# tsinghua-fib-lab/CLSR

Hardware: AMD Instinct MI355X
Metric: train interactions/sec @ batch 4096 seq_len 50 (higher is better)
Workload: dtype f32 (every product at fp32 accuracy: fp32-input MFMAs or three bf16 pieces per operand; the two-piece split-product step is precision_modes.fp32x3)

## Files before the change

### clsr_amd/csrc/linear.hip

```cpp
#include <stdlib.h>
#include "common.h"
#include "clsr_hip.h"
#include <cstdlib>

struct PGemmArgs {
  const float* X; int ldx;
  int T; int G;
  const float* Xmul; int ldmul;
  const float* in_scale; const float* in_shift; int in_relu;
  const float* Wt; int Kp;
  int ldw;
  const float* bias;
  const float* addU; int ldu;
  const float* addV; int ldv;
  float* Y; int ldy; int accumulate;
  double* stats;
  int M, K, N;
  const float* ez; int ldez; const float* e_scale; const float* e_shift; const float* e_mean; const float* e_invstd;
  int no_ring;
  int no_compact;
  int rm_tc, rm_T, rm_t0;
};

__device__ __forceinline__ int range_row(int v, int rm_tc, int rm_T, int rm_t0) {
  if (rm_tc == 0) return v;
  const int q = (int)((unsigned)v / (unsigned)rm_tc);
  return q * rm_T + rm_t0 + (v - q * rm_tc);
}

template <int OT, bool STATS>
__global__ void __launch_bounds__(256) pgemm_generic_kernel(PGemmArgs a) {
  extern __shared__ __attribute__((aligned(16))) float lds[];
  const int tid = threadIdx.x, wave = tid >> 6, lane = tid & 63;
  const int j = lane & 15, g = lane >> 4;
  const int ntile_out = (a.N + 15) >> 4;
// ... 701 lines not shown
  for (int e = blockIdx.x * 256 + threadIdx.x; e < total; e += gridDim.x * 256) {
    const int o = e / d.I, i = e - o * d.I;
    float v = d.s1 * (d.transposed ? d.src1[(long)o * d.ld1 + i] : d.src1[(long)i * d.ld1 + o]);
    if (d.src2) v += d.s2 * (d.transposed ? d.src2[(long)o * d.ld2 + i] : d.src2[(long)i * d.ld2 + o]);
    d.dst[(long)(d.o0 + o) * d.Kp + d.i0 + i] = v;
  }
}

extern "C" int clsr_sizeof_pack_desc(void) { return (int)sizeof(clsr_pack_desc); }

extern "C" int clsr_pack_batch(const clsr_pack_desc* descs_device, int n, int max_elems, void* stream) {
  CLSR_CHECK_ARG(descs_device && n > 0 && max_elems > 0);
  int bx = clsr_cdiv(max_elems, 256);
  if (bx > 64) bx = 64;
  hipLaunchKernelGGL(pack_batch_kernel, dim3(bx, n), dim3(256), 0, (hipStream_t)stream, descs_device);
  CLSR_CHECK_LAUNCH();
  return CLSR_OK;
}

#define DW_T CLSR_DW_T
#define DW_CHUNK CLSR_DW_CHUNK

struct DwArgs {
  const void* X; int ldx; int T; int G; const float* Xmul; int ldmul;
  const float* in_scale; const float* in_shift; int in_relu;
  const void* dY; int ldy;
  float* partial;
  int M, K, N;
  int rm_tc, rm_T, rm_t0, pstride, poff;
};

#define DW_W (16 * DW_T)
#define DW_LDS_FLOATS (64 * 2 * DW_W > 2 * DW_CHUNK ? 64 * 2 * DW_W : 2 * DW_CHUNK)
template <int MODE, bool XH = false, bool YH = false, int KTC = 0, int NTC = 0>
__device__ __forceinline__ void dw_body(const DwArgs& a, float* lds, const int bx, const int gx, const int by,
                                        const int bz, const int gz) {
  float* Xs = lds;
  float* Ys = lds + 64 * DW_W;
  const int tid = threadIdx.x, wave = tid >> 6, lane = tid & 63;
  const int i = lane & 15, g = lane >> 4;
  const int k0 = by * DW_W, n0 = bz * DW_W;
  const int ktc = KTC ? KTC : min(DW_T, ((a.K + 15) >> 4) - by * DW_T);
  const int ntc = NTC ? NTC : min(DW_T, ((a.N + 15) >> 4) - bz * DW_T);
  const int kmax4 = ((a.K + 3) & ~3) - 4, nmax4 = a.N - 4;

  f32x4 acc[DW_T][DW_T];
#pragma unroll
  for (int kt = 0; kt < DW_T; ++kt)
#pragma unroll
    for (int nt = 0; nt < DW_T; ++nt) acc[kt][nt] = (f32x4){0.f, 0.f, 0.f, 0.f};
  float bsum[DW_T];
#pragma unroll
  for (int nt = 0; nt < DW_T; ++nt) bsum[nt] = 0.f;

  constexpr int Q = DW_W / 4;
  constexpr int NLD = 64 * Q / 256;
  f32x4 xr[NLD], yr[NLD], mr[MODE == 1 ? NLD : 1];
  unsigned vmask = 0;
  f32x4 scv[MODE == 2 ? NLD : 1], shv[MODE == 2 ? NLD : 1];
  if (MODE == 2) {
#pragma unroll
    for (int j = 0; j < NLD; ++j) {
      const int idx = tid + 256 * j;
      const int c4 = idx - (idx / Q) * Q;
      int kcol = k0 + 4 * c4;
      kcol = kcol <= kmax4 ? kcol : kmax4;
      scv[j] = ld4(a.in_scale + kcol);
// ... 12 lines not shown
      m = range_row(m < a.M ? m : a.M - 1, a.rm_tc, a.rm_T, a.rm_t0);
      int kcol = k0 + 4 * c4, ncol = n0 + 4 * c4;
      if (mv && kcol <= kmax4) vmask |= 1u << j;
      if (mv && ncol <= nmax4) vmask |= 1u << (8 + j);
      kcol = kcol <= kmax4 ? kcol : kmax4;
      ncol = ncol <= nmax4 ? ncol : nmax4;
      long xrow = m, r = m;
      if (a.T > 0) {
        const unsigned rr = (unsigned)m / (unsigned)a.T;
        r = rr;
        if (a.G > 0) xrow = (long)(rr / (unsigned)a.G) * a.T + (m - (int)rr * a.T);
      }
      xr[j] = load4e<XH>(a.X, xrow * a.ldx + kcol);
      if (MODE == 1) mr[j] = ld4(a.Xmul + r * a.ldmul + kcol);
      yr[j] = load4e<YH>(a.dY, (long)m * a.ldy + ncol);
    }
  };
  auto stage = [&]() {
    const f32x4 z = {0.f, 0.f, 0.f, 0.f};
#pragma unroll
    for (int j = 0; j < NLD; ++j) {
      const int idx = tid + 256 * j;
      f32x4 xv = xr[j];
      if (MODE == 1) xv *= mr[j];
      if (MODE == 2) {
        xv = xv * scv[j] + shv[j];
        if (a.in_relu) { xv.x = fmaxf(xv.x, 0.f); xv.y = fmaxf(xv.y, 0.f); xv.z = fmaxf(xv.z, 0.f); xv.w = fmaxf(xv.w, 0.f); }
      }
      st4(Xs + 4 * idx, (vmask >> j) & 1u ? xv : z);
      st4(Ys + 4 * idx, (vmask >> (8 + j)) & 1u ? yr[j] : z);
    }
  };

  fetch(bx);
  for (int tile = bx; tile < ntiles; tile += gx) {
    __syncthreads();
    stage();
    __syncthreads();
    fetch(tile + gx);
    const float* xw = Xs + (16 * wave + g) * DW_W + i;
    const float* yw = Ys + (16 * wave + g) * DW_W + i;
#pragma unroll
    for (int s = 0; s < 4; ++s) {
      float av[DW_T], bv[DW_T];
#pragma unroll
      for (int t = 0; t < DW_T; ++t) {
        av[t] = xw[(4 * s) * DW_W + 16 * t];
        bv[t] = yw[(4 * s) * DW_W + 16 * t];
      }
#pragma unroll
      for (int kt = 0; kt < DW_T; ++kt)
        if (kt < ktc) {
#pragma unroll
          for (int nt = 0; nt < DW_T; ++nt)
            if (nt < ntc) MFMA4(acc[kt][nt], av[kt], bv[nt]);
        }
#pragma unroll
      for (int nt = 0; nt < DW_T; ++nt) bsum[nt] += bv[nt];
    }
  }
#pragma unroll
  for (int nt = 0; nt < DW_T; ++nt) bsum[nt] = col4_sum(bsum[nt]);
  __syncthreads();
  float* red = lds;

  auto store_to = [&](float* dst) {
// ... 8 lines not shown
    if (g == 0) {
#pragma unroll
      for (int nt = 0; nt < DW_T; ++nt) dst[DW_T * DW_T * 256 + nt * 16 + i] = bsum[nt];
    }
  };
  auto add_from = [&](const float* src) {
#pragma unroll
    for (int kt = 0; kt < DW_T; ++kt)
#pragma unroll
      for (int nt = 0; nt < DW_T; ++nt) {
        const float* t = src + (kt * DW_T + nt) * 256 + (4 * g) * 16 + i;
        acc[kt][nt] += (f32x4){t[0], t[16], t[32], t[48]};
      }
#pragma unroll
    for (int nt = 0; nt < DW_T; ++nt) bsum[nt] += src[DW_T * DW_T * 256 + nt * 16 + i];
  };
  if (wave >= 2) store_to(red + (wave - 2) * DW_CHUNK);
  __syncthreads();
  if (wave < 2) add_from(red + wave * DW_CHUNK);
  __syncthreads();
  if (wave == 1) store_to(red);
  __syncthreads();
  if (wave == 0) {
    add_from(red);
    const long chunk = (long)by * gz + bz;
    store_to(a.partial + (chunk * a.pstride + a.poff + bx) * DW_CHUNK);
  }
}

template <int MODE, bool XH = false, bool YH = false, int KTC = 0, int NTC = 0>
__global__ void __launch_bounds__(256) pgemm_dw_kernel(DwArgs a) {
  __shared__ __attribute__((aligned(16))) float lds[DW_LDS_FLOATS];
  dw_body<MODE, XH, YH, KTC, NTC>(a, lds, blockIdx.x, gridDim.x, blockIdx.y, blockIdx.z, gridDim.z);
}

#define DWM_MAX 12
struct DwMultiArgs {
  DwArgs d[DWM_MAX];
  int first[DWM_MAX + 1];
  int gx[DWM_MAX];
  short nch[DWM_MAX];
  short mode[DWM_MAX];
  int n;
  int spec;
};
__global__ void __launch_bounds__(256) dw_multi_kernel(DwMultiArgs m) {
  __shared__ __attribute__((aligned(16))) float lds[DW_LDS_FLOATS];
  int j = 0;
  while (j + 1 < m.n && (int)blockIdx.x >= m.first[j + 1]) ++j;
  const int local = blockIdx.x - m.first[j];
  const int gx = m.gx[j], nch = m.nch[j];
  const int bx = local % gx, c = local / gx;
  const int by = c / nch, bz = c - by * nch;
  const int ktc = min(DW_T, ((m.d[j].K + 15) >> 4) - by * DW_T), ntc = min(DW_T, ((m.d[j].N + 15) >> 4) - bz * DW_T);
  if (m.mode[j] == 0) {
    if (m.spec && ktc == 3 && ntc == 5) dw_body<0, false, false, 3, 5>(m.d[j], lds, bx, gx, by, bz, nch);
    else if (m.spec && ktc == 5 && ntc == 5) dw_body<0, false, false, 5, 5>(m.d[j], lds, bx, gx, by, bz, nch);
    else if (m.spec > 1 && ktc == 5 && ntc == 3) dw_body<0, false, false, 5, 3>(m.d[j], lds, bx, gx, by, bz, nch);
    else dw_body<0>(m.d[j], lds, bx, gx, by, bz, nch);
  } else if (m.mode[j] == 1) {
    if (m.spec > 1 && ktc == 3 && ntc == 3) dw_body<1, false, false, 3, 3>(m.d[j], lds, bx, gx, by, bz, nch);
    else dw_body<1>(m.d[j], lds, bx, gx, by, bz, nch);
  } else dw_body<2>(m.d[j], lds, bx, gx, by, bz, nch);
}

__global__ void __launch_bounds__(1024) dw_reduce_kernel(const float* __restrict__ partial, int nparts, int K,
                                                        int N, int kchunks, int nchunks, float scale,
                                                        float* __restrict__ dW, int ldw,
                                                        float* __restrict__ db, int accumulate) {
  __shared__ float red[16][64];
  const int total = K * N + (db ? N : 0);
  const int e = blockIdx.x * 64 + (threadIdx.x & 63);
  const int sub = threadIdx.x >> 6;
  float s = 0.f;
  float* o = nullptr;
  if (e < total) {
    const float* p;
    if (e < K * N) {
      const int k = e / N, n = e - k * N;
      const int kc = k / (16 * DW_T), nc = n / (16 * DW_T);
      const int kk = k - kc * 16 * DW_T, nn = n - nc * 16 * DW_T;
      const long off = ((kk >> 4) * DW_T + (nn >> 4)) * 256 + (kk & 15) * 16 + (nn & 15);
      p = partial + ((long)(kc * nchunks + nc) * nparts) * DW_CHUNK + off;
      o = dW + (long)k * ldw + n;
    } else {
      const int n = e - K * N;
      const int nc = n / (16 * DW_T), nn = n - nc * 16 * DW_T;
      p = partial + ((long)nc * nparts) * DW_CHUNK + DW_T * DW_T * 256 + nn;
      o = db + n;
    }
    for (int w = sub; w < nparts; w += 16) s += p[(long)w * DW_CHUNK];
  }
  red[sub][threadIdx.x & 63] = s;
  __syncthreads();
  if (sub == 0 && e < total) {
    s = 0.f;
#pragma unroll
    for (int u = 0; u < 16; ++u) s += red[u][threadIdx.x];
    s *= scale;
    *o = accumulate ? *o + s : s;
  }
}

static int dw_grid_x(int M) {
  int tiles = clsr_cdiv(M, 64);
  int gx = clsr_cdiv(tiles, 4);
  constexpr int cap = 512;
  if (gx > cap) gx = cap;
  if (gx < 1) gx = 1;
  return gx;
}

extern "C" long clsr_pgemm_dw_workspace_floats(int M, int K, int N) {
  const long chunks = (long)clsr_cdiv(K, 16 * DW_T) * clsr_cdiv(N, 16 * DW_T);
  return chunks * dw_grid_x(M) * DW_CHUNK;
}

static int dw_launch_partial(const void* X, int ldx, int T, int G, const float* Xmul, int ldmul,
                             const float* in_scale, const float* in_shift, int in_relu, const void* dY, int ldy,
                             int M, int K, int N, float* workspace, hipStream_t s, int* gx_out, int x_bf16 = 0,
                             int dy_bf16 = 0) {
  CLSR_CHECK_ARG(X && dY && workspace && M >= 0 && K > 0 && N > 0);
  CLSR_CHECK_ARG(!(in_scale && !in_shift));
  CLSR_CHECK_SUPPORTED(N % 4 == 0 && ldx % 4 == 0 && ldy % 4 == 0 && ldx >= ((K + 3) & ~3) &&
                       (!Xmul || (ldmul % 4 == 0 && ldmul >= ((K + 3) & ~3))) &&
                       ((uintptr_t)X % 16) == 0 && ((uintptr_t)dY % 16) == 0);
  DwArgs a;
  a.X = X; a.ldx = ldx; a.T = T; a.G = G; a.Xmul = Xmul; a.ldmul = ldmul;
  a.in_scale = in_scale; a.in_shift = in_shift; a.in_relu = in_relu;
  a.dY = dY; a.ldy = ldy; a.partial = workspace; a.M = M; a.K = K; a.N = N;
  const int kch = clsr_cdiv(K, 16 * DW_T), nch = clsr_cdiv(N, 16 * DW_T);
  const int gx = dw_grid_x(M);
  a.rm_tc = a.rm_T = a.rm_t0 = 0; a.pstride = gx; a.poff = 0;
  CLSR_CHECK_SUPPORTED(!(Xmul && in_scale) && !(in_scale && K % 4));
  if (x_bf16 || dy_bf16) {
    CLSR_CHECK_SUPPORTED(dy_bf16 && ((x_bf16 && in_scale) || (!x_bf16 && Xmul)));
    if (x_bf16) hipLaunchKernelGGL((pgemm_dw_kernel<2, true, true>), dim3(gx, kch, nch), dim3(256), 0, s, a);
    else hipLaunchKernelGGL((pgemm_dw_kernel<1, false, true>), dim3(gx, kch, nch), dim3(256), 0, s, a);
    CLSR_CHECK_LAUNCH();
    *gx_out = gx;
    return CLSR_OK;
  }
  const int ktn = clsr_cdiv(K, 16), ntn = clsr_cdiv(N, 16);
  const bool one = kch == 1 && nch == 1;
#define DW_SPEC(MD, KT_, NT_)                                                                                          \
  if (one && ktn == KT_ && ntn == NT_) {                                                                               \
    hipLaunchKernelGGL((pgemm_dw_kernel<MD, false, false, KT_, NT_>), dim3(gx, 1, 1), dim3(256), 0, s, a);            \
    CLSR_CHECK_LAUNCH();                                                                                               \
    *gx_out = gx;                                                                                                      \
    return CLSR_OK;                                                                                                    \
  }
  if (Xmul) { DW_SPEC(1, 5, 5) DW_SPEC(1, 3, 3) }
  else if (in_scale) { DW_SPEC(2, 5, 3) DW_SPEC(2, 5, 5) }
  else { DW_SPEC(0, 5, 5) DW_SPEC(0, 3, 5) DW_SPEC(0, 3, 3) DW_SPEC(0, 5, 3) }
#undef DW_SPEC
  if (Xmul) hipLaunchKernelGGL(pgemm_dw_kernel<1>, dim3(gx, kch, nch), dim3(256), 0, s, a);
  else if (in_scale) hipLaunchKernelGGL(pgemm_dw_kernel<2>, dim3(gx, kch, nch), dim3(256), 0, s, a);
  else hipLaunchKernelGGL(pgemm_dw_kernel<0>, dim3(gx, kch, nch), dim3(256), 0, s, a);
  CLSR_CHECK_LAUNCH();
  *gx_out = gx;
  return CLSR_OK;
}

extern "C" int clsr_sizeof_dwjob(void) { return (int)sizeof(clsr_dwjob); }

extern "C" int clsr_pgemm_dw_partial_multi(const clsr_dwjob* jobs, int n, void* stream) {
  CLSR_CHECK_ARG(jobs && n > 0 && n <= DWM_MAX);
  DwMultiArgs m;
  m.n = n;
  int total = 0;
  for (int j = 0; j < n; ++j) {
    const clsr_dwjob& q = jobs[j];
    CLSR_CHECK_ARG(q.X && q.dY && q.workspace && q.M > 0 && q.K > 0 && q.N > 0 && !(q.in_scale && !q.in_shift));
    CLSR_CHECK_SUPPORTED(!q.x_bf16 && !q.dy_bf16);
    CLSR_CHECK_SUPPORTED(q.N % 4 == 0 && q.ldx % 4 == 0 && q.ldy % 4 == 0 && q.ldx >= ((q.K + 3) & ~3) &&
                         (!q.Xmul || (q.ldmul % 4 == 0 && q.ldmul >= ((q.K + 3) & ~3))) &&
                         ((uintptr_t)q.X % 16) == 0 && ((uintptr_t)q.dY % 16) == 0);
    CLSR_CHECK_SUPPORTED(!(q.Xmul && q.in_scale) && !(q.in_scale && q.K % 4));
    DwArgs& a = m.d[j];
    a.X = q.X; a.ldx = q.ldx; a.T = q.T; a.G = q.G; a.Xmul = q.Xmul; a.ldmul = q.ldmul;
    a.in_scale = q.in_scale; a.in_shift = q.in_shift; a.in_relu = q.in_relu;
    a.dY = q.dY; a.ldy = q.ldy; a.partial = q.workspace; a.M = q.M; a.K = q.K; a.N = q.N;
    const int kch = clsr_cdiv(q.K, 16 * DW_T), nch = clsr_cdiv(q.N, 16 * DW_T);
    m.first[j] = total;
    m.gx[j] = q.pgx > 0 ? q.pgx : dw_grid_x(q.M);
    CLSR_CHECK_ARG(q.rm_tc >= 0 && (q.rm_tc == 0 || (q.rm_T >= q.rm_t0 + q.rm_tc && q.rm_t0 >= 0 && q.M % q.rm_tc == 0 && !q.T)));
    CLSR_CHECK_ARG(q.pstride == 0 || (q.poff >= 0 && q.poff + m.gx[j] <= q.pstride));
    a.rm_tc = q.rm_tc; a.rm_T = q.rm_T; a.rm_t0 = q.rm_t0;
    a.pstride = q.pstride > 0 ? q.pstride : m.gx[j]; a.poff = q.pstride > 0 ? q.poff : 0;
    m.nch[j] = (short)nch;
    m.mode[j] = (short)(q.Xmul ? 1 : (q.in_scale ? 2 : 0));
    total += m.gx[j] * kch * nch;
  }
  m.first[n] = total;
  m.spec = 2;
  hipLaunchKernelGGL(dw_multi_kernel, dim3(total), dim3(256), 0, (hipStream_t)stream, m);
  CLSR_CHECK_LAUNCH();
  return CLSR_OK;
}

extern "C" int clsr_pgemm_dw(const float* X, int ldx, int T, int G, const float* Xmul, int ldmul,
                             const float* in_scale, const float* in_shift, int in_relu,
                             const float* dY, int ldy, int M, int K, int N, float scale, float* dW,
                             int ldw, float* db, int accumulate, float* workspace, void* stream) {
  CLSR_CHECK_ARG(dW && ldw >= N);
  hipStream_t s = (hipStream_t)stream;
  int gx = 0;
  int rc = dw_launch_partial(X, ldx, T, G, Xmul, ldmul, in_scale, in_shift, in_relu, dY, ldy, M, K, N, workspace, s,
                             &gx);
  if (rc) return rc;
  const int kch = clsr_cdiv(K, 16 * DW_T), nch = clsr_cdiv(N, 16 * DW_T);
  const int total = K * N + (db ? N : 0);
  hipLaunchKernelGGL(dw_reduce_kernel, dim3(clsr_cdiv(total, 64)), dim3(1024), 0, s, workspace, gx, K, N, kch,
                     nch, scale, dW, ldw, db, accumulate);
  CLSR_CHECK_LAUNCH();
  return CLSR_OK;
}

extern "C" int clsr_pgemm_dw_partial(const float* X, int ldx, int T, int G, const float* Xmul, int ldmul,
                                     const float* in_scale, const float* in_shift, int in_relu,
                                     const float* dY, int ldy, int M, int K, int N, float* workspace,
                                     void* stream) {
  int gx = 0;
  return dw_launch_partial(X, ldx, T, G, Xmul, ldmul, in_scale, in_shift, in_relu, dY, ldy, M, K, N, workspace,
                           (hipStream_t)stream, &gx);
}

extern "C" int clsr_pgemm_dw_partial_h(const void* X, int x_bf16, int ldx, int T, int G, const float* Xmul, int ldmul,
                                       const float* in_scale, const float* in_shift, int in_relu,
                                       const void* dY, int dy_bf16, int ldy, int M, int K, int N, float* workspace,
                                       void* stream) {
  int gx = 0;
  return dw_launch_partial(X, ldx, T, G, Xmul, ldmul, in_scale, in_shift, in_relu, dY, ldy, M, K, N, workspace,
                           (hipStream_t)stream, &gx, x_bf16, dy_bf16);
}

extern "C" int clsr_pgemm_dw_parts(int M) { return dw_grid_x(M); }
extern "C" int clsr_sizeof_dw_desc(void) { return (int)sizeof(clsr_dw_desc); }

__global__ void __launch_bounds__(1024) dw_reduce_batch_kernel(const clsr_dw_desc* __restrict__ descs) {
  __shared__ float red[16][64];
  const clsr_dw_desc d = descs[blockIdx.y];
  const int K = d.K, N = d.N;
  const int lane = threadIdx.x & 63, sub = threadIdx.x >> 6;
  const int ktiles = (K + 15) >> 4, ntiles = (N + 15) >> 4;
  const int nchunks = (N + 16 * DW_T - 1) / (16 * DW_T);
  const int wq = ktiles * ntiles * 4;
  const int items = wq + (d.db ? (N + 63) / 64 : 0);
  for (int it = blockIdx.x; it < items; it += gridDim.x) {
    float s = 0.f;
    float* o = nullptr;
    const float* p = nullptr;
    const float* p2 = nullptr;
    if (it < wq) {
      const int tile = it >> 2, q = it & 3;
      const int ktg = tile / ntiles, ntg = tile - ktg * ntiles;
      const int kc = ktg / DW_T, kt = ktg - kc * DW_T, nc = ntg / DW_T, nt = ntg - nc * DW_T;
      const int w = q * 64 + lane;
// ... 45 lines not shown
```

### clsr_amd/net.py

```python
import math
import contextlib
import os
import warnings
from collections import OrderedDict

import numpy as np
import torch

from clsr_amd import ops
from clsr_amd.ops import call, query
from clsr_amd.params import CL, TABLES, UNUSED_TABLE, init_tensor, param_specs

BN_MOMENTUM = 0.95
BN_EPS = 1e-4
F32 = torch.float32


def _pad4(n):
    return (n + 3) // 4 * 4


TF_OPTIMIZERS = {
    "sgd": (0, ()), "gd": (0, ()), "pgd": (0, ()),
    "adagrad": (1, (("accumulator", 0.1),)), "padagrad": (2, (("accumulator", 0.1),)),
# ... 79 lines not shown
        self.att_hist_bwd_pieces = 3 if self.exact_products else 2
        self.bf16_chain = self.precision == "bf16" and os.environ.get("CLSR_BF16_CHAIN", "x1") == "x1"
        self._cur_descs_h = []
        self._plans, self._plan_keep, self._cur_descs = {}, [], []
        self._sort_bytes = {}
        self._ws_tag = ""
        self._side = _SIDE_STREAMS.setdefault(str(torch.device(device)), {})
        self._dense_fork = None
        self._dw_async = False
        self.split_query = True
        self.split_query_min = 16
        self.use_plans = not os.environ.get("CLSR_NO_PLAN")
        self._step_plans = {}
        self._dw_batch = None
        self._buf_allocs = 0
        self.stream_alias = {"@aux": "@lt"}
        self.side_priority = 0
        self.dw_priority = 0
        self.rnn_products = os.environ.get("CLSR_RNN_PRODUCTS", "x6" if self.exact_products else "x3")
        if self.rnn_products not in ("x6", "fp32") + (() if self.exact_products else ("x3",)):
            raise ValueError("CLSR_RNN_PRODUCTS must be 'x6' or 'fp32' (precision='fp32'), also 'x3' otherwise")
        if self.rnn_products == "x6" and max(self.H, self.Du) > 48:
            self.rnn_products = "fp32"
        self.rnn_fused_proj = self.rnn_products in ("x3", "x6") and not os.environ.get("CLSR_NO_RNN_FUSED_PROJ")
        self.proj_gate_pieces = 3 if self.exact_products else 2
        self.proj_bwd_pieces = 3 if self.exact_products else 2
        self.proj_wide_pieces = (2 if self.precision == "bf16" else 3)
        self.rnn_act_tiled = self.rnn_products in ("x3", "x6")
        self.set_att_bwd(os.environ.get("CLSR_ATT_BWD", "x6l1" if self.exact_products else "x3"))
        self.heads_fused = not os.environ.get("CLSR_NO_HEADS_FUSED")
        self.dw_wide = True
        self.dw_wide_entry = (("clsr_pgemm_dw_wide" if os.environ.get("CLSR_DW_WIDE", "x6") == "fp32" else "clsr_pgemm_dw_wide_x6")
                              if self.exact_products else "clsr_pgemm_dw_wide_x3")
        self._dw_batch_wide = None
        self._heads_defer = False
        self._early_lists = None
        self.heads_comm = None
        self._defer_logit_out = False
        self.fold_hist_shares = not os.environ.get("CLSR_NO_FOLD_SHARES")
        self._fold_args, self._folded = None, False
        self.early_user_update = not os.environ.get("CLSR_NO_EARLY_USER_UPDATE")
        self._updated_early = set()
        self._joins = []
        self._dw_pending, self._dw_tables, self._dw_after, self._rp_pending = {}, {}, {}, {}
        self.defer_dw = True
        self.overlap = not os.environ.get("CLSR_NO_OVERLAP")
        self.det_grads = not os.environ.get("CLSR_NO_DET_GRADS")
        self.adam_state = torch.tensor([0.0, 1.0, 1.0, 0.0, 0.0, 0.0, 0.0, 0.0], dtype=torch.float64, device=self.device)
        self.stats24 = torch.zeros(24, dtype=torch.float64, device=self.device)
        self.sumsq_tab, self.losses = self.stats24[:16], self.stats24[16:]
        self.ucount = torch.zeros(1, dtype=F32, device=self.device)
        self.last_shape = None
        self._counts_zeroed = self._ucount_zeroed = self._ticked = False
        self.dp_world = 1
        self.dp_stats_hook = None
        self.dp_comm = None
        self.dp_hooks = None
        self.capture_grads = False
        self.captured = None
        self._aborted = None

    def set_att_bwd(self, mode):
        if mode not in ("x6", "x6l1", "fp32") + (() if self.exact_products else ("x3",)):
            raise ValueError("CLSR_ATT_BWD must be 'x6', 'x6l1' or 'fp32' (precision='fp32'), also 'x3' otherwise")
        self.att_bwd_l0 = "fp32" if mode == "x6l1" else mode
        self.att_bwd = "x6" if mode == "x6l1" else mode
# ... 21 lines not shown
            bad.append("contrastive_loss must be bpr or triplet")
        D = hp.item_embedding_dim + hp.cate_embedding_dim
        if hp.hidden_size != D or hp.user_embedding_dim != D:
            bad.append("hidden_size and user_embedding_dim must equal item+cate dims (alpha fusion, clsr.py:265)")
        bad += self._shape_limits(hp, rnn=True)
        if self.precision == "bf16":
            att = [int(w) for w in hp.att_fcn_layer_sizes]
            qs = (int(hp.user_embedding_dim), int(hp.user_embedding_dim) + D)
            if any(w % 8 for w in att) or any(q % 8 for q in qs) or int(hp.hidden_size) % 8:
                bad.append("precision='bf16' needs att_fcn_layer_sizes %r, the attention query widths %r and hidden_size "
                           "%d to be multiples of 8 (use precision='fp32')" % (att, qs, int(hp.hidden_size)))
        if bad:
            raise NotImplementedError("CLSR HIP path does not support: " + "; ".join(bad))

    @staticmethod
    def _shape_limits(hp, rnn):
        bad = []
        Di, Dc = int(hp.item_embedding_dim), int(hp.cate_embedding_dim)
        if Di % 4 or Dc % 4 or Di <= 0 or Dc <= 0 or Di + Dc > 256:
            bad.append("item / cate embedding dims must be positive multiples of 4, at most 256 together")
        if rnn and (int(hp.hidden_size) % 4 or not 4 <= int(hp.hidden_size) <= 128):
            bad.append("hidden_size must be a multiple of 4 in 4..128")
        if int(hp.max_seq_length) > 256:
            bad.append("max_seq_length must be at most 256")
        widths = list(hp.layer_sizes) + list(getattr(hp, "att_fcn_layer_sizes", None) or [])
        if any(int(w) % 4 or not 4 <= int(w) <= 1024 for w in widths):
            bad.append("MLP layer widths must be multiples of 4 in 4..1024")
        if any(int(w) > 256 for w in (getattr(hp, "att_fcn_layer_sizes", None) or [])):
            bad.append("att_fcn_layer_sizes must be at most 256 wide")
        return bad

    _SWITCHES = ("precision", "table_bf16", "exact_products", "x3", "bf16", "overlap", "defer_dw", "det_grads", "lazy",
                 "use_plans", "heads_fused", "early_user_update", "fold_hist_shares", "enc_x6", "rnn_products", "rnn_fused_proj",
                 "rnn_act_tiled", "att_bwd", "att_bwd_l0", "_l1x", "_l0x", "bf16_chain", "dw_wide", "dw_wide_entry", "split_query",
                 "split_query_min", "rowlist_min_elems", "att_hist_bwd_pieces", "proj_gate_pieces", "proj_bwd_pieces",
                 "proj_wide_pieces")

    def _plan_key(self, what, f):
        hp = self.hp
        g = lambda k: getattr(hp, k, None)
        return (what, id(f), ops.stream_ptr(), self.dp_world, id(self.dp_hooks), id(self.dp_stats_hook), self.dp_comm, self.heads_comm,
                getattr(self, "dp_generation", 0)) + tuple(getattr(self, n, None) for n in self._SWITCHES) + (
                g("learning_rate"), g("embed_l2"), g("layer_l2"), g("embed_l1"), g("layer_l1"), g("max_grad_norm"), g("is_clip_norm"),
                g("discrepancy_loss_weight"), g("contrastive_loss_weight"), g("triplet_margin"),
                g("contrastive_length_threshold"), g("manual_alpha_value"))

    def _planned(self, what, f, run):
        if (not self.use_plans) or self.capture_grads or ops.recording():
            return run()
        key = self._plan_key(what, f)
        ent = self._step_plans.get(key)
        if ent is None:
            self._step_plans[key] = [f, None]
            return run()
        if ent[1] is None:
            plan = ops.record_begin()
            try:
                plan.result = run()
            finally:
                ops.record_end()
            ent[1] = plan
            ent.append(self.last_shape)
            return plan.result
        ops.replay(ent[1])
        self.last_shape = ent[2]
        return ent[1].result

# ... 366 lines not shown
            self._dw_flush()

    def _dw_wide(self, X, ldx, Xmul, ldmul, dY, ldy, M, K, N, dW, ldw, db, acc):
        key = "dww_ws%s.%d.%d.%x" % (self._ws_tag, K, N, dW.data_ptr())
        ws = self._buf(key, query("clsr_pgemm_dw_wide_workspace_floats", M, K, N))
        job = (X, ldx, Xmul, ldmul, dY, ldy, M, K, N, ws, dW, ldw, db, acc)
        if self._dw_batch is not None:
            self._dw_batch_wide.append(job)
            return
        side = None
        if self.overlap and self._ws_tag == "":
            side = self._side_stream("@dw0")
            ops.stream_wait(side, self._fork_point())
            self._dw_async = True
        call(self.dw_wide_entry, *job, stream=side.cuda_stream if side is not None else None)

    @contextlib.contextmanager
    def _dw_batched(self, late=False):
        if not self.defer_dw or self._dw_batch is not None:
            yield
            return
        fork = self._fork_point()
        allocs = self._buf_allocs
        self._dw_batch, self._dw_batch_wide = [], []
        try:
            yield
        finally:
            jobs, self._dw_batch = self._dw_batch, None
            wide, self._dw_batch_wide = self._dw_batch_wide, None
        if not jobs and not wide:
            return
        if late or self._buf_allocs != allocs:
            fork = self._fork_point()
        name = "clsr_hdw_partial_multi" if self.bf16 else "clsr_pgemm_dw_partial_multi"
        if self.overlap and self._ws_tag == "":
            side = self._side_stream("@dw0")
            ops.stream_wait(side, fork)
            if jobs:
                ops.dw_multi(name, jobs, stream=side.cuda_stream)
            for job in wide:
                call(self.dw_wide_entry, *job, stream=side.cuda_stream)
            self._dw_async = True
        else:
            if jobs:
                ops.dw_multi(name, jobs)
            for job in wide:
                call(self.dw_wide_entry, *job)

    def _dw_parts_query(self, any_bf16=False):
        return "clsr_hdw_parts" if self.bf16 else "clsr_pgemm_dw_parts"

    def _dw_launch(self, X, x_bf16, ldx, T, G, Xmul, ldmul, sc, sh, dY, dy_bf16, ldy, M, K, N, ws, stream):
        if self.bf16:
            call("clsr_hdw_partial", X, x_bf16, ldx, T, G, Xmul, ldmul, sc, sh, 1, dY, dy_bf16, ldy, M, K, N, ws,
                 stream=stream)
        elif x_bf16 or dy_bf16:
            call("clsr_pgemm_dw_partial_h", X, x_bf16, ldx, T, G, Xmul, ldmul, sc, sh, 1, dY, dy_bf16, ldy, M, K, N, ws,
                 stream=stream)
        else:
            call("clsr_pgemm_dw_partial", X, ldx, T, G, Xmul, ldmul, sc, sh, 1, dY, ldy, M, K, N, ws, stream=stream)

    def _dw_fused(self, ws, parts, K, N, dW, ldw, db=None, acc=0):
        self._dw_pending.setdefault(self._ws_tag, []).append(
            (ws.data_ptr(), dW.data_ptr(), db.data_ptr() if db is not None else 0, 1.0, parts, K, N, ldw, acc))
        if not self.defer_dw:
            self._dw_flush()

    def _rp(self, partial, parts, stride, n, out):
        self._rp_pending.setdefault(self._ws_tag, []).append(
            (partial.data_ptr(), out.data_ptr(), 1.0, parts, stride, n, 0, 0))

    def _dw_flush(self, tag=None):
        tag = self._ws_tag if tag is None else tag
        pend = self._dw_pending.pop(tag, [])
        if tag == "" and self._dw_async:
            cur = ops.current_stream()
            side = self._side.get("@dw0")
            if side is not None and side.cuda_stream != cur.cuda_stream:
                ops.stream_wait(cur, ops.event_record(side))
            self._dw_async = False
        if pend:
            sig = tuple(pend)
            tab = self._dw_tables.get(sig)
            if tab is None:
                tab = self._dw_tables[sig] = ops.dw_table(sig, self.device)
            call("clsr_dw_reduce_batch", tab[0], tab[1], tab[2])
        rp = self._rp_pending.pop(tag, [])
        if rp:
            ops.multi("clsr_reduce_parts_multi", ops.RpDesc, rp)
        for fn in self._dw_after.pop(tag, []):
            fn()

    def _stats_buf(self, M, N):
# ... 1590 lines not shown
            ops.multi("clsr_tables_reg_multi" + self._th, ops.TableDesc, sweep, l2e, l1e, self.ucount, self.losses[1:])
        if self.capture_grads:
            self.captured = dict(dense={n: g.detach().clone() for n, g in self.Gd.items()},
                                 tables={k: g.detach().clone() for k, g in tg.items()},
                                 dense_sumsq=self.dense_sumsq.clone(), table_sumsq=ss.clone())
            call("clsr_adam_tick", self.adam_state, float(hp.learning_rate), 0.9, 0.999)
            self._dense_update(clip)
        if not tick_early:
            self._join()
        rest = []
        for key, partner, slot, dscale, dloss_scale, dloss, base, nsum in spec:
            V, C = tb[key].shape
            if key in lists and self.tf_opt is not None:
                ids, count, cap = lists[key]
                call("clsr_table_tf_rows", self.tf_opt[0], tb[key], tg[key], self.tab_m.get(key), self.tab_v.get(key),
                     fl[key], ids, count, cap, C, ss[base:], 2, nsum, clip, self.adam_state, lr)
            elif key in lists and self.lazy:
                ids, count, cap = lists[key]
                call("clsr_table_adam_rows" + self._th, tb[key], tg[key], self.tab_m[key], self.tab_v[key], fl[key], ids, count,
                     cap, C, ss[base:], 2, nsum, clip, self.adam_state, 0.9, 0.999, 1e-8)
            elif key in lists:
                call("clsr_table_adam" + self._th, tb[key], tg[key], self.tab_m[key], self.tab_v[key], fl[key], V, C, ss[base:],
                     2, nsum, clip, self.adam_state, 0.9, 0.999, 1e-8, self.lazy)
            else:
                rest.append(key)
        if rest:
            self._tables_update_multi([r for r in sweep if r[0] in {tb[k].data_ptr() for k in rest}], clip)
        if tick_early:
            self._join()

    def precision_note(self):
        if self.precision == "fp32":
            return ("all tensors fp32; EVERY product at fp32 accuracy: v_mfma_f32_16x16x4_f32 (bit-exact fp32 fma chains: recurrences, "
                    "layer-0 forward, heads, encoder-side weight gradients) or three bf16 pieces per operand on "
                    "v_mfma_f32_16x16x32_bf16 with fp32 accumulation (2^-23 relative: history-level attention forward / backward, "
                    "layer-1 forward, the attention-MLP backward with its folded weight gradients%s, the Time4LSTM time-gate "
                    "projection); no two-piece (2^-16) product anywhere" % ("" if self.att_bwd == "x6" else " [CLSR_ATT_BWD=fp32: fp32 MFMAs]"))
        if self.precision == "fp32x3":
            return ("all tensors fp32 (storage, statistics, losses, optimiser exactly as in the fp32 mode); forward products in front "
                    "of a batch-norm + ReLU at fp32 accuracy; the recurrences' hidden products, the attention-MLP backward with its "
                    "folded weight gradients, the history-level attention backward and the fused encoder tail as TWO-piece split-bf16 "
                    "sums hi*hi + hi*lo + lo*hi on v_mfma_f32_16x16x32_bf16 with fp32 accumulation (2^-16 relative per product "
                    "term: narrower than the reference's fp32 products)")
        return ("attention-block activations at (row, step) level (z0, z1, dz0) stored as bf16, their products with ONE bf16 piece per "
                "operand on v_mfma_f32_16x16x32_bf16 with fp32 accumulation"
                + (" (the parity mode's chain kernels with the weight gradients folded in, csrc/attbwdx3.hip)" if self.bf16_chain
                   else " (position-tiled csrc/hgemm.hip kernels, CLSR_BF16_CHAIN=old)")
                + "; history- and row-level tensors, batch-norm statistics, softmax, recurrences, losses, gradients of the "
                "parameters and the optimiser stay fp32")

    def bench_att_layer0(self, f, time_kernel):
        B, T, G, Hn = self.last_shape
        Qs, A0 = self.Du + self.D, self.A0
        run = self._att_layer0_launcher("st", Hn, G, T, Qs)
        t_mm = time_kernel(run)
        flops = 2.0 * B * T * Qs * A0
        bf = self.precision == "bf16"
        peak = 2500.0 if bf else 157.3
        if bf and self._bf16_chain_ok(G, Qs):
            nbytes = float(B) * T * A0 * 2 + float(Hn) * T * (Qs + A0) * 4 + float(B) * (Qs + A0) * 4
            return dict(bound="hbm", kernel="att_l0_fwd_kernel<5,5,1,bf16> (short-term attention layer 0, one wave per history, one "
                                            "bf16 piece per operand, bf16 z0)",
                        achieved=round(nbytes / t_mm / 1e9, 1), peak=8000.0, unit="GB/s", frac=round(nbytes / t_mm / 8e12, 4),
                        bytes_per_launch=nbytes, us_per_launch=round(t_mm * 1e6, 2),
                        formula="B*T*A0*2 (bf16 z0 written) + Hn*T*(Q + A0)*4 (a, U read) + B*(Q + A0)*4 (q, V read)",
                        mfma_tflops=round(flops / t_mm / 1e12, 2))
        return dict(bound="mfma", kernel=(("hgemm_l0g_kernel (short-term attention layer 0, bf16 MFMA, one wave per history group)"
                                           if query("clsr_hgemm_l0_group_supported", G, Qs, A0) else
                                           "hgemm_kernel<MUL,UV> (short-term attention layer 0, bf16 MFMA)") if bf else
                                          "att_l0_fwd_kernel<5,5> (short-term attention layer 0, one wave per history)"
# ... 114 lines not shown
```

### include/clsr_hip.h

```cpp
#ifndef CLSR_HIP_H
#define CLSR_HIP_H
#include <stddef.h>
#ifdef __cplusplus
extern "C" {
#endif

int clsr_version(void);
int clsr_last_error(char* buf, size_t n);

int clsr_graph_begin(void* stream);
int clsr_graph_end(void* stream, void** graph_exec_out);
int clsr_graph_launch(void* graph_exec, void* stream);
int clsr_graph_destroy(void* graph_exec);

int clsr_gather_hist_fwd(const float* item_tbl, const float* cate_tbl, const int* item_idx,
                         const int* cate_idx, long idx_row_stride, const int* seq_len, int len_stride,
                         int Hn, int T, int Di, int Dc, int recent_k, float* hist, float* hist_mean,
                         float* hist_recent, void* stream);
int clsr_gather_hist_fwd_h(const void* item_tbl, const void* cate_tbl, const int* item_idx,
                           const int* cate_idx, long idx_row_stride, const int* seq_len, int len_stride,
                           int Hn, int T, int Di, int Dc, int recent_k, void* hist, int hist_bf16,
                           float* hist_mean, float* hist_recent, void* stream);
int clsr_gather_rows(const float* tbl, const int* idx, long idx_stride, int N, int C, float* out,
                     int ldo, int col0, void* stream);
// ... 273 lines not shown
int clsr_hgemm_l0_group_stats_parts(long Hn);
int clsr_hgemm_l0_group(const float* a, int lda, const float* q, int ldq, const void* Wt, int Kp,
                        const float* U, int ldu, const float* V, int ldv, void* z0, int ldz, double* stats,
                        long Hn, int G, int T, int Q, int A0, void* stream);
int clsr_hgemm_hf32(const void* X, int ldx, const void* Wt, int Kp, float* Y, int ldy, int accumulate,
                    int M, int K, int N, void* stream);
int clsr_pgemm_stats_parts(int M);
int clsr_pgemm_range(const float* X, int ldx, const float* Wt, int Kp, const float* bias, float* Y, int ldy,
                     int accumulate, int Hn, int T, int t0, int t1, int K, int N, void* stream);
int clsr_pgemm(const float* X, int ldx, int T, int G, const float* Xmul, int ldmul,
               const float* in_scale, const float* in_shift, int in_relu, const float* Wt, int Kp,
               const float* bias, const float* addU, int ldu, const float* addV, int ldv, float* Y,
               int ldy, int accumulate, double* stats, int M, int K, int N, void* stream);
int clsr_pgemm_bnbwd(const float* X, int ldx, const float* Wt, int Kp, float* Y, int ldy, const float* z,
                     int ldz, const float* scale, const float* shift, const float* mean, const float* invstd,
                     double* stats, int M, int K, int N, void* stream);
long clsr_pgemm_dw_workspace_floats(int M, int K, int N);
int clsr_pgemm_dw(const float* X, int ldx, int T, int G, const float* Xmul, int ldmul,
                  const float* in_scale, const float* in_shift, int in_relu, const float* dY, int ldy,
                  int M, int K, int N, float scale, float* dW, int ldw, float* db, int accumulate,
                  float* workspace, void* stream);
typedef struct clsr_dw_desc {
  const float* partial; float* dW; float* db;
  float scale;
  int nparts; int K; int N; int ldw; int accumulate;
  const float* partial2; float scale2; int nparts2;
} clsr_dw_desc;
int clsr_sizeof_dw_desc(void);
int clsr_pgemm_dw_parts(int M);
int clsr_hdw_parts(int M);
int clsr_pgemm_dw_partial(const float* X, int ldx, int T, int G, const float* Xmul, int ldmul,
                          const float* in_scale, const float* in_shift, int in_relu, const float* dY, int ldy,
                          int M, int K, int N, float* workspace, void* stream);
int clsr_dw_reduce_batch(const clsr_dw_desc* descs_device, int n, int max_outputs, void* stream);

int clsr_sum_parts_d(const double* partial, int nparts, int n, double* out, void* stream);
int clsr_bn_finalize(const double* stats_partial, int nparts, int C, double count, const float* gamma,
                     const float* beta, float* moving_mean, float* moving_var, float momentum, float eps,
                     int training, float* scale, float* shift, float* mean_out, float* invstd_out,
                     void* stream);
int clsr_colred_parts(int M, int C);
int clsr_bn_relu_bwd_reduce(float* dh, const float* z, const float* scale, const float* shift,
                            const float* mean, const float* invstd, int M, int C, double* partial,
                            void* stream);
int clsr_bn_bwd_coef(const double* partial, int nparts, int C, double count, const float* gamma,
                     const float* mean, const float* invstd, float* coef, float* dgamma, float* dbeta,
                     int accumulate, void* stream);
int clsr_bn_bwd_coef_scaled(const double* partial, int nparts, int C, double count, const float* gamma,
                            const float* mean, const float* invstd, float* coef, float* dgamma, float* dbeta,
                            int accumulate, double grad_scale, void* stream);
int clsr_bn_bwd_apply(float* dy, const float* z, const float* coef, long M, int C, void* stream);
int clsr_bn_bwd_coef_apply(const double* partial, int nparts, int C, double count, const float* gamma,
                           const float* mean, const float* invstd, float* coef, float* dgamma, float* dbeta,
                           float* dy, const float* z, long M, void* stream);

int clsr_att_out_fwd(const float* z1, const float* scale1, const float* shift1, const float* w_out,
                     const float* b_out, const int* seq_len, int len_stride, const float* keys, int Hn,
                     int G, int T, int C1, int Dk, float* wts, float* out, void* stream);
int clsr_att_score_bwd_parts(int Hn);
int clsr_att_score_bwd(const float* dout, const float* wts, const int* seq_len, int len_stride,
                       const float* keys, int Hn, int G, int T, int Dk, float* ds, float* dkeys,
                       float* b_partial, void* stream);
int clsr_att_dy1_parts(long M, int C1);
int clsr_att_dy1_stats(const float* z1, const float* ds, const float* scale1, const float* shift1,
                       const float* mean1, const float* invstd1, const float* w_out, long M, int C1,
                       double* bn_partial, float* w_partial, void* stream);
// ... 175 lines not shown
int clsr_stage_feed(void* dst, const void* src_host, long nbytes, void* stream);
int clsr_copy_words(void* dst, const void* src, long nbytes, void* stream);

#define CLSR_MULTI_MAX 16
typedef struct clsr_mark_desc { const int* idx; unsigned char* flags; long nrows; long row_stride; int ncols; int pad_; } clsr_mark_desc;
typedef struct clsr_gather_desc { const float* table; const int* idx; float* out; long idx_stride; int N; int C; int ldo; int col0; } clsr_gather_desc;
int clsr_enc_bwd_fused_supported(int D, int n, int NX);
int clsr_enc_bwd_fused_parts(long M);
long clsr_enc_bwd_fused_workspace_floats(long M, int product);
int clsr_enc_bwd_fused_h_parts(long M);
long clsr_enc_bwd_fused_h_workspace_floats(long M, int product);
int clsr_enc_bwd_fused_h(const void* dPin_bf16, const float* hist, const float* hprev1, const float* gates1,
                         const float* mprev, const float* TT, const float* hprev2, const float* gates2,
                         float* ws_hist, float* ws_hp1, float* ws_hp1r, float* ws_mprev, float* ws_tt,
                         float* ws_hp2, float* ws_hp2r, const void* Wt_bf16, int Kph, float* dhist, long M, void* stream);
int clsr_enc_bwd_fused(const float* dPin, const float* hist, const float* hprev1, const float* gates1,
                       const float* mprev, const float* TT, const float* hprev2, const float* gates2,
                       const float* Wt, int Kp, float* dhist, float* ws_hist, float* ws_hp1, float* ws_hp1r,
                       float* ws_mprev, float* ws_tt, float* ws_hp2, float* ws_hp2r, long M, void* stream);
int clsr_enc_bwd_fused_fold(const float* dPin, const float* hist, const float* hprev1, const float* gates1,
                            const float* mprev, const float* TT, const float* hprev2, const float* gates2,
                            const float* Wt, int Kp, float* dhist, const float* dhist2, const float* dmean,
                            const float* drecent, const int* seq_len, int len_stride, int T, int recent_k,
                            float* ws_hist, float* ws_hp1, float* ws_hp1r, float* ws_mprev, float* ws_tt, float* ws_hp2,
                            float* ws_hp2r, long M, void* stream);

typedef struct clsr_dwjob {
  const void* X; const float* Xmul; const float* in_scale; const float* in_shift; const void* dY; float* workspace;
  int x_bf16; int ldx; int T; int G; int ldmul; int in_relu; int dy_bf16; int ldy; int M; int K; int N; int pad_;
  int rm_tc; int rm_T; int rm_t0; int pgx; int pstride; int poff;
} clsr_dwjob;
int clsr_sizeof_dwjob(void);
int clsr_pgemm_dw_partial_multi(const clsr_dwjob* jobs_host, int n, void* stream);
int clsr_hdw_partial_multi(const clsr_dwjob* jobs_host, int n, void* stream);
typedef struct clsr_rp_desc { const float* partial; float* out; float scale; int nparts; int stride; int n; int accumulate; int pad_; } clsr_rp_desc;
typedef struct clsr_table_desc {
  float* table; const float* partner; float* grad; float* m; float* v; unsigned char* flags;
  double* sumsq_reg; double* disc_loss; const double* sumsq_adam;
  long V; int C; int nsum; int sumsq_stride; float disc_scale; float disc_loss_scale; int pad_;
} clsr_table_desc;
typedef struct clsr_zero_desc { void* p; long nbytes; } clsr_zero_desc;
int clsr_sizeof_zero_desc(void);
int clsr_zero_multi(const clsr_zero_desc* descs_host, int n, void* stream);
typedef struct clsr_scatter_desc {
  const float* src; const int* idx; float* tbl_grad; double* sumsq; long idx_stride; int ld_src; int col0; int N; int C;
} clsr_scatter_desc;
int clsr_sizeof_scatter_desc(void);
int clsr_scatter_add_rows_multi(const clsr_scatter_desc* descs_host, int n, void* stream);
int clsr_sizeof_multi_descs(int* mark, int* gather, int* rp, int* table);
int clsr_mark_rows_multi(const clsr_mark_desc* descs_host, int n, void* stream);
int clsr_gather_rows_multi(const clsr_gather_desc* descs_host, int n, void* stream);
int clsr_gather_rows_multi_h(const clsr_gather_desc* descs_host, int n, void* stream);
int clsr_reduce_parts_multi(const clsr_rp_desc* descs_host, int n, void* stream);
int clsr_tables_reg_multi(const clsr_table_desc* descs_host, int n, float l2, float l1, const float* ucount,
                          double* reg_loss, void* stream);
int clsr_tables_reg_multi_h(const clsr_table_desc* descs_host, int n, float l2, float l1, const float* ucount,
                            double* reg_loss, void* stream);
int clsr_tables_adam_multi(const clsr_table_desc* descs_host, int n, float clip_norm, const double* adam_state,
                           float beta1, float beta2, float eps, int lazy, void* stream);
int clsr_tables_adam_multi_h(const clsr_table_desc* descs_host, int n, float clip_norm, const double* adam_state,
                             float beta1, float beta2, float eps, int lazy, void* stream);
int clsr_tf_opt_slots(int opt);
int clsr_dense_tf(int opt, float* param, float* grad, float* s1, float* s2, const int* seg_of, const unsigned char* skip,
                  const double* sumsq, float clip_norm, const double* state, float lr, int n, void* stream);
int clsr_tables_tf_multi(const clsr_table_desc* descs_host, int n, int opt, float clip_norm, const double* state,
                         float lr, void* stream);
// ... 21 lines not shown
```

Measured before the change: 1.321 million.

## Compute separate weight-gradient products with three-piece bf16 MFMAs instead of fp32 MFMAs

Adds a piece-product path to the weight-gradient partial kernel. Each fp32 operand is split into three bf16 pieces and the six significant cross products are accumulated on bf16 MFMAs in fp32. Waves are rearranged so two wave pairs each take half of the rows and half of one tile dimension, and the two halves are reduced through LDS. The path is enabled by default in exact-products mode through the new x6 entry points. The aim is to raise matrix throughput over the fp32 16x16x4 MFMA, at the cost of extra splitting arithmetic, more register pressure and lower accuracy than fp32 FMA.

After: 1.326 million (median of 6 runs). Within noise of the previous version (+0.4%).

```diff
diff --git a/clsr_amd/csrc/linear.hip b/clsr_amd/csrc/linear.hip
--- a/clsr_amd/csrc/linear.hip
+++ b/clsr_amd/csrc/linear.hip
@@ -1,6 +1,7 @@
 #include <stdlib.h>
 #include "common.h"
 #include "clsr_hip.h"
+#include "hmma.h"
 #include <cstdlib>
 
 struct PGemmArgs {
@@ -768,7 +769,7 @@
 
 #define DW_W (16 * DW_T)
 #define DW_LDS_FLOATS (64 * 2 * DW_W > 2 * DW_CHUNK ? 64 * 2 * DW_W : 2 * DW_CHUNK)
-template <int MODE, bool XH = false, bool YH = false, int KTC = 0, int NTC = 0>
+template <int MODE, bool XH = false, bool YH = false, int KTC = 0, int NTC = 0, int NP = 0>
 __device__ __forceinline__ void dw_body(const DwArgs& a, float* lds, const int bx, const int gx, const int by,
                                         const int bz, const int gz) {
   float* Xs = lds;
@@ -847,6 +848,114 @@
     }
   };
 
+  if constexpr (NP > 0) {
+    static_assert(!XH && !YH, "piece products: fp32 operands");
+    constexpr bool SN = NTC > KTC;
+    constexpr int HT = KTC ? ((SN ? NTC : KTC) + 1) / 2 : 3;
+    const int h = wave >> 1, p = wave & 1;
+    const int mb = p ? HT : 0;
+    const int scnt = SN ? ktc : ntc;
+    const int hcnt = p ? (SN ? ntc : ktc) : min(HT, SN ? ntc : ktc);
+    const int hend = p ? DW_T : HT;
+    f32x4 acc3[3][DW_T];
+#pragma unroll
+    for (int u = 0; u < 3; ++u)
+#pragma unroll
+      for (int v = 0; v < DW_T; ++v) acc3[u][v] = (f32x4){0.f, 0.f, 0.f, 0.f};
+    auto sum8 = [](const f32x8& v) { return ((v[0] + v[1]) + (v[2] + v[3])) + ((v[4] + v[5]) + (v[6] + v[7])); };
+    fetch(bx);
+    for (int tile = bx; tile < ntiles; tile += gx) {
+      __syncthreads();
+      stage();
+      __syncthreads();
+      fetch(tile + gx);
+      const float* hw = (SN ? Ys : Xs) + (32 * h + g) * DW_W + 16 * mb + i;
+      const float* sw = (SN ? Xs : Ys) + (32 * h + g) * DW_W + i;
+      bf16x8 hp[NP][3];
+#pragma unroll
+      for (int u = 0; u < 3; ++u)
+        if (mb + u < hcnt) {
+          f32x8 v;
+#pragma unroll
+          for (int e = 0; e < 8; ++e) v[e] = hw[(4 * e) * DW_W + 16 * u];
+          if (SN) bsum[u] += sum8(v);
+#pragma unroll
+          for (int q = 0; q < NP; ++q) {
+            hp[q][u] = to_h(v);
+            if (q + 1 < NP) v -= to_f(hp[q][u]);
+          }
+        }
+#pragma unroll
+      for (int v = 0; v < DW_T; ++v)
+        if (v < scnt) {
+          f32x8 w;
+#pragma unroll
+          for (int e = 0; e < 8; ++e) w[e] = sw[(4 * e) * DW_W + 16 * v];
+          if (!SN && p) bsum[v] += sum8(w);
+          bf16x8 sp[NP];
+#pragma unroll
+          for (int q = 0; q < NP; ++q) {
+            sp[q] = to_h(w);
+            if (q + 1 < NP) w -= to_f(sp[q]);
+          }
+#pragma unroll
+          for (int sum = NP - 1; sum >= 0; --sum)
+#pragma unroll
+            for (int qa = sum; qa >= 0; --qa)
+#pragma unroll
+              for (int u = 0; u < 3; ++u)
+                if (mb + u < hcnt) {
+                  if (SN) HMFMA(acc3[u][v], sp[qa], hp[sum - qa][u]);
+                  else HMFMA(acc3[u][v], hp[qa][u], sp[sum - qa]);
+                }
+        }
+    }
+#pragma unroll
+    for (int nt = 0; nt < DW_T; ++nt) bsum[nt] = col4_sum(bsum[nt]);
+    __syncthreads();
+    auto tile_at = [&](int u, int v) { return SN ? v * DW_T + mb + u : (mb + u) * DW_T + v; };
+    auto store3 = [&](float* dst) {
+#pragma unroll
+      for (int u = 0; u < 3; ++u)
+        if (mb + u < hend) {
+#pragma unroll
+          for (int v = 0; v < DW_T; ++v) {
+            float* t = dst + tile_at(u, v) * 256 + (4 * g) * 16 + i;
+            const f32x4 c = acc3[u][v];
+            t[0] = c.x; t[16] = c.y; t[32] = c.z; t[48] = c.w;
+          }
+          if (SN && g == 0) dst[DW_T * DW_T * 256 + (mb + u) * 16 + i] = bsum[u];
+        }
+      if (!SN && p && g == 0) {
+#pragma unroll
+        for (int v = 0; v < DW_T; ++v) dst[DW_T * DW_T * 256 + v * 16 + i] = bsum[v];
+      }
+    };
+    auto add3 = [&](const float* src) {
+#pragma unroll
+      for (int u = 0; u < 3; ++u)
+        if (mb + u < hend) {
+#pragma unroll
+          for (int v = 0; v < DW_T; ++v) {
+            const float* t = src + tile_at(u, v) * 256 + (4 * g) * 16 + i;
+            acc3[u][v] += (f32x4){t[0], t[16], t[32], t[48]};
+          }
+          if (SN) bsum[u] += src[DW_T * DW_T * 256 + (mb + u) * 16 + i];
+        }
+      if (!SN && p) {
+#pragma unroll
+        for (int v = 0; v < DW_T; ++v) bsum[v] += src[DW_T * DW_T * 256 + v * 16 + i];
+      }
+    };
+    if (h == 1) store3(lds);
+    __syncthreads();
+    if (h == 0) {
+      add3(lds);
+      const long chunk = (long)by * gz + bz;
+      store3(a.partial + (chunk * a.pstride + a.poff + bx) * DW_CHUNK);
+    }
+    return;
+  }
   fetch(bx);
   for (int tile = bx; tile < ntiles; tile += gx) {
     __syncthreads();
@@ -921,6 +1030,12 @@
 __global__ void __launch_bounds__(256) pgemm_dw_kernel(DwArgs a) {
   __shared__ __attribute__((aligned(16))) float lds[DW_LDS_FLOATS];
   dw_body<MODE, XH, YH, KTC, NTC>(a, lds, blockIdx.x, gridDim.x, blockIdx.y, blockIdx.z, gridDim.z);
+}
+
+template <int NP, int MODE, int KTC = 0, int NTC = 0>
+__global__ void __launch_bounds__(256, 2) pgemm_dw_xp_kernel(DwArgs a) {
+  __shared__ __attribute__((aligned(16))) float lds[DW_LDS_FLOATS];
+  dw_body<MODE, false, false, KTC, NTC, NP>(a, lds, blockIdx.x, gridDim.x, blockIdx.y, blockIdx.z, gridDim.z);
 }
 
 #define DWM_MAX 12
@@ -953,6 +1068,26 @@
   } else dw_body<2>(m.d[j], lds, bx, gx, by, bz, nch);
 }
 
+__global__ void __launch_bounds__(256, 2) dw_multi_x6_kernel(DwMultiArgs m) {
+  __shared__ __attribute__((aligned(16))) float lds[DW_LDS_FLOATS];
+  int j = 0;
+  while (j + 1 < m.n && (int)blockIdx.x >= m.first[j + 1]) ++j;
+  const int local = blockIdx.x - m.first[j];
+  const int gx = m.gx[j], nch = m.nch[j];
+  const int bx = local % gx, c = local / gx;
+  const int by = c / nch, bz = c - by * nch;
+  const int ktc = min(DW_T, ((m.d[j].K + 15) >> 4) - by * DW_T), ntc = min(DW_T, ((m.d[j].N + 15) >> 4) - bz * DW_T);
+  if (m.mode[j] == 0) {
+    if (ktc == 3 && ntc == 5) dw_body<0, false, false, 3, 5, 3>(m.d[j], lds, bx, gx, by, bz, nch);
+    else if (ktc == 5 && ntc == 5) dw_body<0, false, false, 5, 5, 3>(m.d[j], lds, bx, gx, by, bz, nch);
+    else if (ktc == 5 && ntc == 3) dw_body<0, false, false, 5, 3, 3>(m.d[j], lds, bx, gx, by, bz, nch);
+    else dw_body<0, false, false, 0, 0, 3>(m.d[j], lds, bx, gx, by, bz, nch);
+  } else if (m.mode[j] == 1) {
+    if (ktc == 3 && ntc == 3) dw_body<1, false, false, 3, 3, 3>(m.d[j], lds, bx, gx, by, bz, nch);
+    else dw_body<1, false, false, 0, 0, 3>(m.d[j], lds, bx, gx, by, bz, nch);
+  } else dw_body<2, false, false, 0, 0, 3>(m.d[j], lds, bx, gx, by, bz, nch);
+}
+
 __global__ void __launch_bounds__(1024) dw_reduce_kernel(const float* __restrict__ partial, int nparts, int K,
                                                         int N, int kchunks, int nchunks, float scale,
                                                         float* __restrict__ dW, int ldw,
@@ -1008,7 +1143,7 @@
 static int dw_launch_partial(const void* X, int ldx, int T, int G, const float* Xmul, int ldmul,
                              const float* in_scale, const float* in_shift, int in_relu, const void* dY, int ldy,
                              int M, int K, int N, float* workspace, hipStream_t s, int* gx_out, int x_bf16 = 0,
-                             int dy_bf16 = 0) {
+                             int dy_bf16 = 0, int pieces = 0) {
   CLSR_CHECK_ARG(X && dY && workspace && M >= 0 && K > 0 && N > 0);
   CLSR_CHECK_ARG(!(in_scale && !in_shift));
   CLSR_CHECK_SUPPORTED(N % 4 == 0 && ldx % 4 == 0 && ldy % 4 == 0 && ldx >= ((K + 3) & ~3) &&
@@ -1032,6 +1167,26 @@
   }
   const int ktn = clsr_cdiv(K, 16), ntn = clsr_cdiv(N, 16);
   const bool one = kch == 1 && nch == 1;
+  if (pieces) {
+    CLSR_CHECK_SUPPORTED(pieces == 3);
+#define DW_SPEC(MD, KT_, NT_)                                                                                          \
+  if (one && ktn == KT_ && ntn == NT_) {                                                                               \
+    hipLaunchKernelGGL((pgemm_dw_xp_kernel<3, MD, KT_, NT_>), dim3(gx, 1, 1), dim3(256), 0, s, a);                    \
+    CLSR_CHECK_LAUNCH();                                                                                               \
+    *gx_out = gx;                                                                                                      \
+    return CLSR_OK;                                                                                                    \
+  }
+    if (Xmul) { DW_SPEC(1, 5, 5) DW_SPEC(1, 3, 3) }
+    else if (in_scale) { DW_SPEC(2, 5, 3) DW_SPEC(2, 5, 5) }
+    else { DW_SPEC(0, 5, 5) DW_SPEC(0, 3, 5) DW_SPEC(0, 3, 3) DW_SPEC(0, 5, 3) }
+#undef DW_SPEC
+    if (Xmul) hipLaunchKernelGGL((pgemm_dw_xp_kernel<3, 1>), dim3(gx, kch, nch), dim3(256), 0, s, a);
+    else if (in_scale) hipLaunchKernelGGL((pgemm_dw_xp_kernel<3, 2>), dim3(gx, kch, nch), dim3(256), 0, s, a);
+    else hipLaunchKernelGGL((pgemm_dw_xp_kernel<3, 0>), dim3(gx, kch, nch), dim3(256), 0, s, a);
+    CLSR_CHECK_LAUNCH();
+    *gx_out = gx;
+    return CLSR_OK;
+  }
 #define DW_SPEC(MD, KT_, NT_)                                                                                          \
   if (one && ktn == KT_ && ntn == NT_) {                                                                               \
     hipLaunchKernelGGL((pgemm_dw_kernel<MD, false, false, KT_, NT_>), dim3(gx, 1, 1), dim3(256), 0, s, a);            \
@@ -1053,7 +1208,7 @@
 
 extern "C" int clsr_sizeof_dwjob(void) { return (int)sizeof(clsr_dwjob); }
 
-extern "C" int clsr_pgemm_dw_partial_multi(const clsr_dwjob* jobs, int n, void* stream) {
+static int dw_multi_any(const clsr_dwjob* jobs, int n, int pieces, void* stream) {
   CLSR_CHECK_ARG(jobs && n > 0 && n <= DWM_MAX);
   DwMultiArgs m;
   m.n = n;
@@ -1083,9 +1238,16 @@
   }
   m.first[n] = total;
   m.spec = 2;
-  hipLaunchKernelGGL(dw_multi_kernel, dim3(total), dim3(256), 0, (hipStream_t)stream, m);
+  if (pieces) hipLaunchKernelGGL(dw_multi_x6_kernel, dim3(total), dim3(256), 0, (hipStream_t)stream, m);
+  else hipLaunchKernelGGL(dw_multi_kernel, dim3(total), dim3(256), 0, (hipStream_t)stream, m);
   CLSR_CHECK_LAUNCH();
   return CLSR_OK;
+}
+extern "C" int clsr_pgemm_dw_partial_multi(const clsr_dwjob* jobs, int n, void* stream) {
+  return dw_multi_any(jobs, n, 0, stream);
+}
+extern "C" int clsr_pgemm_dw_partial_multi_x6(const clsr_dwjob* jobs, int n, void* stream) {
+  return dw_multi_any(jobs, n, 3, stream);
 }
 
 extern "C" int clsr_pgemm_dw(const float* X, int ldx, int T, int G, const float* Xmul, int ldmul,
@@ -1113,6 +1275,15 @@
   int gx = 0;
   return dw_launch_partial(X, ldx, T, G, Xmul, ldmul, in_scale, in_shift, in_relu, dY, ldy, M, K, N, workspace,
                            (hipStream_t)stream, &gx);
+}
+
+extern "C" int clsr_pgemm_dw_partial_x6(const float* X, int ldx, int T, int G, const float* Xmul, int ldmul,
+                                        const float* in_scale, const float* in_shift, int in_relu,
+                                        const float* dY, int ldy, int M, int K, int N, float* workspace,
+                                        void* stream) {
+  int gx = 0;
+  return dw_launch_partial(X, ldx, T, G, Xmul, ldmul, in_scale, in_shift, in_relu, dY, ldy, M, K, N, workspace,
+                           (hipStream_t)stream, &gx, 0, 0, 3);
 }
 
 extern "C" int clsr_pgemm_dw_partial_h(const void* X, int x_bf16, int ldx, int T, int G, const float* Xmul, int ldmul,
diff --git a/clsr_amd/net.py b/clsr_amd/net.py
--- a/clsr_amd/net.py
+++ b/clsr_amd/net.py
@@ -135,6 +135,7 @@
         self.dw_wide = True
         self.dw_wide_entry = (("clsr_pgemm_dw_wide" if os.environ.get("CLSR_DW_WIDE", "x6") == "fp32" else "clsr_pgemm_dw_wide_x6")
                               if self.exact_products else "clsr_pgemm_dw_wide_x3")
+        self.dw_x6 = self.exact_products and os.environ.get("CLSR_DW", "x6") != "fp32"
         self._dw_batch_wide = None
         self._heads_defer = False
         self._early_lists = None
@@ -222,7 +223,7 @@
 
     _SWITCHES = ("precision", "table_bf16", "exact_products", "x3", "bf16", "overlap", "defer_dw", "det_grads", "lazy",
                  "use_plans", "heads_fused", "early_user_update", "fold_hist_shares", "enc_x6", "rnn_products", "rnn_fused_proj",
-                 "rnn_act_tiled", "att_bwd", "att_bwd_l0", "_l1x", "_l0x", "bf16_chain", "dw_wide", "dw_wide_entry", "split_query",
+                 "rnn_act_tiled", "att_bwd", "att_bwd_l0", "_l1x", "_l0x", "bf16_chain", "dw_wide", "dw_wide_entry", "dw_x6", "split_query",
                  "split_query_min", "rowlist_min_elems", "att_hist_bwd_pieces", "proj_gate_pieces", "proj_bwd_pieces",
                  "proj_wide_pieces")
 
@@ -655,7 +656,8 @@
             return
         if late or self._buf_allocs != allocs:
             fork = self._fork_point()
-        name = "clsr_hdw_partial_multi" if self.bf16 else "clsr_pgemm_dw_partial_multi"
+        name = ("clsr_hdw_partial_multi" if self.bf16 else
+                "clsr_pgemm_dw_partial_multi_x6" if self.dw_x6 else "clsr_pgemm_dw_partial_multi")
         if self.overlap and self._ws_tag == "":
             side = self._side_stream("@dw0")
             ops.stream_wait(side, fork)
@@ -681,7 +683,8 @@
             call("clsr_pgemm_dw_partial_h", X, x_bf16, ldx, T, G, Xmul, ldmul, sc, sh, 1, dY, dy_bf16, ldy, M, K, N, ws,
                  stream=stream)
         else:
-            call("clsr_pgemm_dw_partial", X, ldx, T, G, Xmul, ldmul, sc, sh, 1, dY, ldy, M, K, N, ws, stream=stream)
+            call("clsr_pgemm_dw_partial_x6" if self.dw_x6 else "clsr_pgemm_dw_partial", X, ldx, T, G, Xmul, ldmul, sc, sh, 1,
+                 dY, ldy, M, K, N, ws, stream=stream)
 
     def _dw_fused(self, ws, parts, K, N, dW, ldw, db=None, acc=0):
         self._dw_pending.setdefault(self._ws_tag, []).append(
@@ -2338,10 +2341,13 @@
     def precision_note(self):
         if self.precision == "fp32":
             return ("all tensors fp32; EVERY product at fp32 accuracy: v_mfma_f32_16x16x4_f32 (bit-exact fp32 fma chains: recurrences, "
-                    "layer-0 forward, heads, encoder-side weight gradients) or three bf16 pieces per operand on "
+                    "layer-0 forward, heads%s) or three bf16 pieces per operand on "
                     "v_mfma_f32_16x16x32_bf16 with fp32 accumulation (2^-23 relative: history-level attention forward / backward, "
                     "layer-1 forward, the attention-MLP backward with its folded weight gradients%s, the Time4LSTM time-gate "
-                    "projection); no two-piece (2^-16) product anywhere" % ("" if self.att_bwd == "x6" else " [CLSR_ATT_BWD=fp32: fp32 MFMAs]"))
+                    "projection%s); no two-piece (2^-16) product anywhere"
+                    % ("" if self.dw_x6 else ", every separate weight-gradient product [CLSR_DW=fp32]",
+                       "" if self.att_bwd == "x6" else " [CLSR_ATT_BWD=fp32: fp32 MFMAs]",
+                       ", every separate weight-gradient product (clsr_pgemm_dw_partial_x6)" if self.dw_x6 else ""))
         if self.precision == "fp32x3":
             return ("all tensors fp32 (storage, statistics, losses, optimiser exactly as in the fp32 mode); forward products in front "
                     "of a batch-norm + ReLU at fp32 accuracy; the recurrences' hidden products, the attention-MLP backward with its "
diff --git a/include/clsr_hip.h b/include/clsr_hip.h
--- a/include/clsr_hip.h
+++ b/include/clsr_hip.h
@@ -329,6 +329,9 @@
 int clsr_pgemm_dw_partial(const float* X, int ldx, int T, int G, const float* Xmul, int ldmul,
                           const float* in_scale, const float* in_shift, int in_relu, const float* dY, int ldy,
                           int M, int K, int N, float* workspace, void* stream);
+int clsr_pgemm_dw_partial_x6(const float* X, int ldx, int T, int G, const float* Xmul, int ldmul,
+                             const float* in_scale, const float* in_shift, int in_relu, const float* dY, int ldy,
+                             int M, int K, int N, float* workspace, void* stream);
 int clsr_dw_reduce_batch(const clsr_dw_desc* descs_device, int n, int max_outputs, void* stream);
 
 int clsr_sum_parts_d(const double* partial, int nparts, int n, double* out, void* stream);
@@ -570,6 +573,7 @@
 } clsr_dwjob;
 int clsr_sizeof_dwjob(void);
 int clsr_pgemm_dw_partial_multi(const clsr_dwjob* jobs_host, int n, void* stream);
+int clsr_pgemm_dw_partial_multi_x6(const clsr_dwjob* jobs_host, int n, void* stream);
 int clsr_hdw_partial_multi(const clsr_dwjob* jobs_host, int n, void* stream);
 typedef struct clsr_rp_desc { const float* partial; float* out; float scale; int nparts; int stride; int n; int accumulate; int pad_; } clsr_rp_desc;
 typedef struct clsr_table_desc {
```
